# dropbox/lepton

Hardware: AMD Instinct MI355X
Metric: encode+decode MB/s (JPEG bytes/sec), bit-exact round trip (higher is better)
Workload: dtype int16/u8 (integer coder, no floating point)

## Files before the change

lepton_amd/csrc/lep_dec4.h:

```cpp
#pragma once
#include "lep_v3.h"
#include "lep_enc3.h"

namespace lep4 {
using namespace lep3;

#if LEP_ON_GPU && defined(LEP_MARKS)
#define LEP_MARK(name) __asm__ volatile("; MARK " name)
#elif LEP_ON_GPU && defined(LEP_PROF)
#define LEP_MARK(name) prof_stamp(lep4::prof_slot(name))
#else
#define LEP_MARK(name) ((void)0)
#endif
#if LEP_ON_GPU && (defined(LEP_DEC4_PAD_VALU) || defined(LEP_DEC4_PAD_SALU) || defined(LEP_DEC4_PAD_LDS))
#define LEP_PAD8(x) x x x x x x x x
WDEV void pad_block(uint32_t seed, const void* lds) {
    (void)seed; (void)lds;
#ifdef LEP_DEC4_PAD_VALU
    { uint32_t o; for (int i = 0; i < LEP_DEC4_PAD_VALU / 8; ++i) __asm__ volatile(LEP_PAD8("v_add_u32 %0, %1, %1\n") : "=v"(o) : "v"(seed)); }
#endif
#ifdef LEP_DEC4_PAD_SALU
    { uint32_t o; const uint32_t u = uni(seed); for (int i = 0; i < LEP_DEC4_PAD_SALU / 8; ++i) __asm__ volatile(LEP_PAD8("s_add_u32 %0, %1, %1\n") : "=s"(o) : "s"(u) : "scc"); }
#endif
#ifdef LEP_DEC4_PAD_LDS
// ... 238 lines not shown
#if !LEP_DEC4_REFILL_GROUPS
        if (count < 0) refill(b);
#else
        (void)b;
#endif
#ifdef LEP_DEC4_RANGE_LOW
        const uint32_t split = 1 + (((range - 1) * (pk & 255u)) >> 8);
        const uint32_t big = split << 24;
        uint32_t was = vhi;
        const uint32_t bit = was >= big ? 1u : 0u;
        vhi = bit ? was - big : was;
        range = bit ? range - split : split;
        const int shift = __builtin_clz(range) - 24;
#else
        const uint32_t big = ((uint32_t)(((uint64_t)(range - 0x01000000u) * (uint64_t)(pk << 24)) >> 32) & 0xff000000u) + 0x01000000u;
        uint32_t was = vhi;
        const uint32_t bit = was >= big ? 1u : 0u;
        vhi = bit ? was - big : was;
        range = bit ? range - big : big;
        const int shift = __builtin_clz(range);
#endif
#ifdef LEP_TRACE_GET
        LEP_TRACE_GET(pk & 255u, (int)bit);
#endif
        range <<= shift;
        const uint64_t v = pair64(vhi, vlo) << shift;
        vhi = (uint32_t)(v >> 32); vlo = (uint32_t)v;
        count -= shift;
#if LEP_ON_GPU && !defined(LEP_DEC4_PAIR_OR)
        __asm__ volatile("" : "+s"(was));
        return was >= big ? 1u : 0u;
#else
        return bit;
#endif
    }
};

#ifndef LEP_DEC4_PRIO
#define LEP_DEC4_PRIO 1
#endif
#if LEP_ON_GPU && LEP_DEC4_PRIO
#define LEP_PRIO_SERIAL(on_scalar_unit) __builtin_amdgcn_s_setprio((on_scalar_unit) ? 0 : 1)
#define LEP_PRIO_PARALLEL() __builtin_amdgcn_s_setprio(2)
#else
#define LEP_PRIO_SERIAL(on_scalar_unit) ((void)0)
#define LEP_PRIO_PARALLEL() ((void)0)
#endif
#ifndef LEP_DEC4_SCALAR
#define LEP_DEC4_SCALAR 2
#endif

#ifndef LEP_DEC4_WORD_PER_LANE
#define LEP_DEC4_WORD_PER_LANE 1
#endif

enum : int32_t { kRowsFresh = 0, kRowsRunning = 1, kRowsFinished = 2, kRowsFailed = 3 };
struct Dec4Resume {
    int32_t state, code;
    uint32_t idx, top;
    uint32_t vhi, vlo;
    int32_t count;
    uint32_t range, wi;
    uint32_t nbins;
    int32_t rows_done[3];
    int32_t fail_component, fail_y, fail_x;
};

struct RowsWalk {
    const Dec4Resume* rec; const uint32_t* lds_save;
    bool fresh;
    uint32_t idx, stop, total;
    int band;
    bool top[3];
    int rows_done[3];
    int state, fail_component, fail_y, fail_x;
};

template <int SCMASK>
struct Dec4WaveT {
    const ImageDev* img;
    uint32_t* model;
    Dec4Shared* sh;
    int comp, ci;
    BoolDec4 bc;
    uint32_t nbins;
#if LEP_ON_GPU && !defined(LEP_COUNT_BINS)
#define LEP_BINS(expr) ((void)0)
#else
#define LEP_BINS(expr) (expr)
#endif
#if LEP_ON_GPU && defined(LEP_PROF)
    uint64_t prof_last;
    unsigned long long* prof_out;
    int prof_cur;
    uint32_t prof_acc[20];
    template <int I> __device__ __forceinline__ void prof_add(uint32_t dt) { if (prof_cur == I) prof_acc[I] += dt; }
    __device__ __forceinline__ void prof_stamp(int slot) {
        const uint64_t t = __builtin_readcyclecounter();
        const uint32_t dt = (uint32_t)(t - prof_last);
        prof_last = t;
        prof_add<0>(dt); prof_add<1>(dt); prof_add<2>(dt); prof_add<3>(dt); prof_add<4>(dt); prof_add<5>(dt); prof_add<6>(dt);
        prof_add<7>(dt); prof_add<8>(dt); prof_add<9>(dt); prof_add<10>(dt); prof_add<11>(dt); prof_add<12>(dt); prof_add<13>(dt);
        prof_add<14>(dt); prof_add<15>(dt); prof_add<16>(dt); prof_add<17>(dt); prof_add<18>(dt);
        prof_cur = slot;
    }
    __device__ __forceinline__ void prof_begin(unsigned long long* out) {
// ... 178 lines not shown
#define LEP_SLOT(k, fld)                                                                                              \
        if (!((kAlways >> k) & 1)) { LANES(l) L(any) = (L(used) >> k) & 1; }                                           \
        if (((kAlways >> k) & 1) || lepwave::wave_ballot(any)) {                                                       \
            LANES(l) {                                                                                                \
                const uint32_t w = L(W).fld;                                                                          \
                const uint32_t u1 = ((uint32_t)(L(used) & L(bits)) >> k) & 1u, u0 = ((uint32_t)(L(used) & ~L(bits)) >> k) & 1u;   \
                const uint32_t w2 = w + (u0 | (u1 << 8));                                                             \
                const uint32_t f = w2 & 255u, t = (w2 >> 8) & 255u;                                                   \
                const uint32_t p = mul24_low(f, inv[f + t]);    \
                const uint32_t m = mul24(u0 | u1, 0xff0000u);                                                         \
                L(oldw) = w; L(low) = (f < t ? f : t) + ((u0 | u1) ^ 1u);    \
                L(W).fld = (p & m) | (w2 & ~m);                                                                       \
            }                                                                                                         \
            LANES(l) L(any) = L(low) == 0;                                                                            \
            if (lepwave::wave_ballot(any)) {                                                                          \
                LANES(l) if (L(low) == 0) L(W).fld = bupd_t(L(oldw), (uint32_t)(L(bits) >> k) & 1u, inv);             \
            }                                                                                                         \
        }
        LEP_SLOT(0, x) LEP_SLOT(1, y) LEP_SLOT(2, z) LEP_SLOT(3, w)
#undef LEP_SLOT
    }

    WDEV void adapt_words(uint32_t* W, const int* use, const int* obs) {
        const uint32_t* inv = sh->inv24;
        LV(int, wrapped); LV(uint32_t, oldw);
        LANES(l) {
            const uint32_t w = L(W);
            const uint32_t u = (uint32_t)L(use), u1 = u & (uint32_t)L(obs), u0 = u & ~(uint32_t)L(obs);
            const uint32_t w2 = w + (u0 | (u1 << 8));
            const uint32_t f = w2 & 255u, t = (w2 >> 8) & 255u;
            const uint32_t p = mul24_low(f, inv[f + t]);
            const uint32_t m = mul24(u, 0xff0000u);
            L(oldw) = w; L(wrapped) = (f < t ? f : t) + (u ^ 1u) == 0;
            L(W) = (p & m) | (w2 & ~m);
        }
        if (lepwave::wave_ballot(wrapped)) {
            LANES(l) if (L(wrapped)) L(W) = bupd_t(L(oldw), (uint32_t)L(obs), inv);
        }
    }
    static WDEV void regroup(const U4* G, const int* src, const int* slot, uint32_t* out) {
        LV(uint32_t, c0); LV(uint32_t, c1); LV(uint32_t, c2); LV(uint32_t, c3);
        LV(uint32_t, g0); LV(uint32_t, g1); LV(uint32_t, g2); LV(uint32_t, g3);
        LANES(l) { L(c0) = L(G).x; L(c1) = L(G).y; L(c2) = L(G).z; L(c3) = L(G).w; }
        lepwave::wave_gather(c0, src, g0); lepwave::wave_gather(c1, src, g1);
        lepwave::wave_gather(c2, src, g2); lepwave::wave_gather(c3, src, g3);
        LANES(l) { const int k = L(slot); L(out) = k == 0 ? L(g0) : (k == 1 ? L(g1) : (k == 2 ? L(g2) : L(g3))); }
    }
    WDEV void adapt_regrouped(const U4* G, const uint32_t* adr, const int* src, const int* slot, const int* use, const int* obs) {
        LV(uint32_t, Wd); LV(uint32_t, ad);
        regroup(G, src, slot, Wd);
        lepwave::wave_gather(adr, src, ad);
        adapt_words(Wd, use, obs);
        LANES(l) if (L(use)) model[L(ad) + (uint32_t)L(slot)] = L(Wd);
    }

    WDEV int round_nz(int nzbin_ctx) {
        LEP_MARK("nz_prefetch");
        LV(U4, W0); LV(uint32_t, a0); LV(uint32_t, PK0);
        LANES(l) {
            uint32_t adr = 0, pk = 0;
            if (l < 17) {
                int i, k;
                if (l < 3) { i = 5 - l; k = 0; } else if (l < 5) { i = 2; k = l - 3; } else if (l < 9) { i = 1; k = l - 5; } else { i = 0; k = l - 9; }
                adr = ctx_nz7(ci, nzbin_ctx) + (uint32_t)i * 32 + (uint32_t)k * 4;
                L(W0) = ld4(model + adr); pk = pack_probs(L(W0));
            }
            L(a0) = adr; L(PK0) = pk;
        }
        LEP_MARK("nz_serial"); LEP_PRIO_SERIAL((SCMASK & 1) != 0);
        int nz;
        {
            Serial<(SCMASK & 1) != 0> sr(*this);
            nz = sr.template tree<6>(PK0, 0);
            sr.done();
            LEP_BINS(nbins += 6);
        }
        LEP_MARK("nz_update"); LEP_PRIO_PARALLEL();
#if LEP_DEC4_WORD_PER_LANE
        {
            LV(int, src); LV(int, slot); LV(int, use); LV(int, ob);
            LANES(l) {
                const int t = l < 6 ? l : 0, i = 5 - t, prefix = nz >> (i + 1);
                L(src) = ((0x953210 >> (4 * t)) & 15) + (prefix >> 2); L(slot) = prefix & 3; L(use) = l < 6; L(ob) = (nz >> i) & 1;
            }
            adapt_regrouped(W0, a0, src, slot, use, ob);
        }
#else
        LV(int, u0); LV(int, b0);
        LANES(l) {
            int u = 0, b = 0;
            if (l < 17) {
                int i, k;
                if (l < 3) { i = 5 - l; k = 0; } else if (l < 5) { i = 2; k = l - 3; } else if (l < 9) { i = 1; k = l - 5; } else { i = 0; k = l - 9; }
                mask_tree(i, k, nz, u, b);
            }
            L(u0) = u; L(b0) = b;
        }
        adapt_group<3>(W0, u0, b0);
        LANES(l) if (L(u0)) st4(model + L(a0), L(W0));
#endif
        return nz;
    }

    WDEV void round_77(int& zz_io, int& left_io) {
        Dec4Shared& S = *sh;
        LEP_MARK("77_prefetch");
// ... 26 lines not shown
        {
            typedef Serial<(SCMASK & 2) != 0> SR;
            SR sr(*this);
            uint32_t sgw = SR::U(S.sign[ci * 48]);
            int pi = 0;
#pragma nounroll
            for (;;) {
                int lane = pi + 16 * cand;
                const int lane_end = pi_end + 16 * cand;
                uint32_t pkv;
                bool found = false;
#pragma nounroll
                for (;;) {
                    pkv = SR::U(lepwave::wave_read(PK0, lane));
                    LEP_BINS(++nbins);
                    if (SR::is(sr.get(pkv & 255) != 0)) { found = true; break; }
                    if (++lane >= lane_end) break;
                }
                pi = lane - 16 * cand;
                if (!found) break;
                zz = zz0 + pi;
                int len = sr.template unary_from<1, false>(pkv);
                if (len == 4) {
                    len = 4 + sr.template unary_from<0>(SR::U(pack_probs(vload4(model + ctx4_exp7(ci, nb0 - cand, zz, (int)uni(S.bsr[zz])) + kGS))));
                    if (len == 8) len = sr.unary_tail(ctx4_exp7(ci, nb0 - cand, zz, (int)uni(S.bsr[zz])));
                }
                LEP_BINS(nbins += (uint32_t)(2 * len - (len == 11)));
                const uint32_t pos = sr.get(sgw >> 16);
                sgw = sr.bupd(sgw, pos);
                --left;
                uint32_t v = 1u << (len - 1);
                if (len > 1) {
                    int b = len - 2;
                    if (b >= 4) {
                        const uint32_t rbase = ctx4_res(ci, (int)uni(S.a2r[zz]), nb0 - cand);
#pragma nounroll
                        for (; b >= 4; --b) v |= sr.global_bin(row_word(rbase, b)) << b;
                    }
                    v = sr.residual(SR::U(lepwave::wave_read(PK1, lane)), b, v);
                }
                S.here[zz] = (int16_t)(pos ? (int)v : -(int)v);
                ++pi;
                if (left == 0) break;
                cand = nb0 - nzbin_of(left);
                if (cand >= LEP_DEC4_CANDS || pi >= pi_end) break;
            }
            zz = zz0 + pi;
            sr.done();
            S.sign[ci * 48] = sgw;
        }
        LSYNC();
        LEP_MARK("77_update"); LEP_PRIO_PARALLEL();
        LV(int, nzw);
        LANES(l) L(nzw) = l < 16 && zz0 + l < zz && S.here[zz0 + l] != 0;
        const uint32_t nzmask = (uint32_t)lepwave::wave_ballot(nzw);
        LV(int, u0); LV(int, b0); LV(int, u1); LV(int, b1); LV(int, u2); LV(int, b2);
#if LEP_DEC4_WORD_PER_LANE
        LV(int, src); LV(int, slot);
        LANES(l) {
            int s = l, ua = 0, oa = 0, ub = 0, ob = 0, uc = 0, bcc = 0;
            const int pi = l & 15, k = l >> 4, p = zz0 + pi;
            if (p < zz) {
                const int left_at = left0 - __builtin_popcount(nzmask & ((1u << pi) - 1));
                const int c = left_at > 0 ? nb0 - (int)S.nzbin[left_at] : LEP_DEC4_CANDS;
                if (c < LEP_DEC4_CANDS) {
                    const int cf = S.here[p];
                    const int v = cf < 0 ? -cf : cf, len = bitlen((uint32_t)v);
                    s = pi + 16 * c;
                    ua = k <= len; oa = len != k;
                    ub = k <= len - 2; ob = (v >> k) & 1;
                    if (c == k) mask_exp(4, len, uc, bcc);
                }
            }
            L(src) = s; L(slot) = k; L(u0) = ua; L(b0) = oa; L(u1) = ub; L(b1) = ob; L(u2) = uc; L(b2) = bcc;
        }
        adapt_regrouped(W0, a0, src, slot, u0, b0);
        if (lepwave::wave_ballot(u1)) adapt_regrouped(W1, a1, src, slot, u1, b1);
#else
        LANES(l) {
            int ua = 0, ba = 0, ub = 0, bb = 0, uc = 0, bcc = 0;
            const int pi = l & 15, cand_l = l >> 4, p = zz0 + pi;
            if (L(ok) && p < zz) {
                const int left_at = left0 - __builtin_popcount(nzmask & ((1u << pi) - 1));
                if (left_at > 0 && nb0 - (int)S.nzbin[left_at] == cand_l) {
                    const int cf = S.here[p];
                    const int v = cf < 0 ? -cf : cf, len = bitlen((uint32_t)v);
                    mask_exp(0, len, ua, ba);
                    mask_res(len - 2, v, ub, bb);
                    mask_exp(4, len, uc, bcc);
                }
            }
            L(u0) = ua; L(b0) = ba; L(u1) = ub; L(b1) = bb; L(u2) = uc; L(b2) = bcc;
        }
        adapt_group<3>(W0, u0, b0);
        adapt_group<0>(W1, u1, b1);
        LANES(l) {
            if (L(u0)) st4(model + L(a0), L(W0));
            if (L(u1)) st4(model + L(a1), L(W1));
        }
#endif
        if (lepwave::wave_ballot(u2)) {
            LV(U4, W2);
            LANES(l) if (L(u2)) L(W2) = ld4(model + L(a0) + kGS);
            adapt_group<0>(W2, u2, b2);
            LANES(l) if (L(u2)) st4(model + L(a0) + kGS, L(W2));
        }
        LSYNC();
        zz_io = zz; left_io = left;
    }

    WDEV int round_edges(int nz, int eob_x, int eob_y, bool has_left, bool has_above) {
        Dec4Shared& S = *sh;
        LEP_MARK("edge_prefetch");
        LV(U4, W0); LV(U4, W1); LV(U4, W2); LV(uint32_t, a0); LV(uint32_t, a2); LV(uint32_t, PK0); LV(uint32_t, PK1); LV(uint32_t, PK2);
        LV(uint32_t, INFO);
        LANES(l) {
            uint32_t adr0 = 0, adr2 = 0, pk0 = 0, pk1 = 0, pk2 = 0, info = 0;
            if (l < 56) {
                const int e = l >= 28 ? 1 : 0, c = l - e * 28, j = S.cj[c], n = S.cn[c];
                const bool horizontal = e == 0;
                const int coord = horizontal ? j + 1 : (j + 1) * 8;
                const int32_t prior = S.eprior[e * 7 + j];
                const uint32_t ap = prior < 0 ? 0u - (uint32_t)prior : (uint32_t)prior;
                const int bsr = bitlen(ap > 1023 ? 1023 : ap);
                adr0 = ctx4_expx(ci, n, horizontal ? j : j + 7, bsr);
                adr2 = ctx4_res(ci, coord, n);
                L(W0) = ld4(model + adr0); L(W2) = ld4(model + adr2);
                pk0 = pack_probs(L(W0)); pk2 = pack_probs(L(W2));
                L(W1) = U4{0, 0, 0, 0};
                const int16_t p16 = (int16_t)prior;
                const int thr = S.thr[coord];
                const uint32_t tctx = (uint32_t)imin((int)((ap & 0xffff) >> thr), 255);
                info = (uint32_t)((ci * 4 + (p16 == 0 ? 0 : (p16 > 0 ? 1 : 2))) * 12 + bsr) | ((uint32_t)thr << 8) | (tctx << 16) |
                       ((uint32_t)bsr << 24) | ((S.eprior[14] >> (e * 7 + j)) & 1 ? 0x80000000u : 0u);
            } else if (l < 62) {
                const int e = l >= 59 ? 1 : 0, lv = l - 56 - 3 * e;
                adr0 = ctx_nzedge(e == 0, ci, e == 0 ? eob_x : eob_y, (nz + 3) / 7) + (uint32_t)(2 - lv) * 4;
                L(W0) = ld4(model + adr0); pk0 = pack_probs(L(W0));
            }
            L(a0) = adr0; L(a2) = adr2; L(PK0) = pk0; L(PK1) = pk1; L(PK2) = pk2; L(INFO) = info;
        }
        LSYNC();
        LEP_MARK("edge_serial"); LEP_PRIO_SERIAL((SCMASK & 4) != 0);
        int ne[2] = {0, 0}, rc = 0;
        typedef Serial<(SCMASK & 4) != 0> SR;
        SR sr(*this);
#pragma nounroll
        for (int e = 0; e < 2 && !rc; ++e) {
            const bool horizontal = e == 0;
            ne[e] = sr.template tree<3>(PK0, 56 + 3 * e);
            LEP_BINS(nbins += 3);
            int left = ne[e];
            if (!left) continue;
            const int a_off = horizontal ? 50 : 57;
            int lane = e * 28 + left - 1, step = 7;
#pragma nounroll
            for (;;) {
                if (SR::is(left > step)) {
#pragma nounroll
// ... 41 lines not shown
                    const int coord = horizontal ? j + 1 : (j + 1) * 8;
                    int len = sr.template unary_from<1, false>(pkv);
                    if (len == 4) {
                        len = 4 + sr.template unary_from<0>(SR::U(pack_probs(vload4(model + ctx4_expx(ci, left, horizontal ? j : j + 7, (int)((info >> 24) & 15)) + kGS))));
                        if (len == 8) len = sr.unary_tail(ctx4_expx(ci, left, horizontal ? j : j + 7, (int)((info >> 24) & 15)));
                    }
                    LEP_BINS(nbins += (uint32_t)(2 * len - (len == 11)));
                    const int sslot = (int)(info & 255);
                    const uint32_t sgw = SR::U(S.sign[sslot]);
                    const uint32_t pos = sr.get(sgw >> 16);
                    S.sign[sslot] = sr.bupd(sgw, pos);
                    uint32_t v = 1u << (len - 1);
                    if (len > 1) {
                        int b = len - 2;
                        const int thr = (int)((info >> 8) & 15);
                        if (b >= thr) {
                            const uint32_t Tt = ctx_thresh(ci, (int)((info >> 16) & 255), imin(len - thr, 7));
                            int sx = 1;
#pragma nounroll
                            for (; b >= thr; --b) {
                                const uint32_t bit = sr.global_bin(Tt + (uint32_t)sx);
                                v |= bit << b;
                                sx = imin((sx << 1) | (int)uni(bit), 127);
                            }
                        }
                        if (b >= 4) {
                            const uint32_t rbase = ctx4_res(ci, coord, left);
#pragma nounroll
                            for (; b >= 4; --b) v |= sr.global_bin(row_word(rbase, b)) << b;
                        }
                        v = sr.residual(SR::U(lepwave::wave_read(PK2, lane)), b, v);
                    }
                    S.here[a_off + j] = (int16_t)(pos ? (int)v : -(int)v);
                    --lane;
                    if (--left == 0) break;
                }
                lane += step;
                if (--step == 0) break;
            }
        }
        sr.done();
        LSYNC();
        if (rc) return rc;
        LEP_MARK("edge_update"); LEP_PRIO_PARALLEL();
        LV(int, enz);
        LANES(l) L(enz) = l >= 50 && S.here[l] != 0;
        const uint64_t em = lepwave::wave_ballot(enz);
        const uint32_t mh = (uint32_t)(em >> 50) & 0x7f, mv = (uint32_t)(em >> 57) & 0x7f;
        const int neh = ne[0], nev = ne[1];
        LV(int, u1); LV(int, b1); LV(int, u2); LV(int, b2);
#if !LEP_DEC4_WORD_PER_LANE
        LV(int, u0); LV(int, b0);
#endif
        LANES(l) {
            int ua = 0, ba = 0, ub = 0, bb = 0, uc = 0, bcc = 0;
            if (l < 56) {
                const int e = l >= 28 ? 1 : 0, c = l - e * 28, j = S.cj[c], n = S.cn[c];
                const uint32_t mk = e ? mv : mh;
                const int left_at = (e ? nev : neh) - __builtin_popcount(mk & ((1u << j) - 1));
                if (left_at == n) {
                    const int cf = S.here[(e ? 57 : 50) + j];
                    const int v = cf < 0 ? -cf : cf, len = bitlen((uint32_t)v);
#if !LEP_DEC4_WORD_PER_LANE
                    mask_exp(0, len, ua, ba);
#endif
                    mask_exp(4, len, ub, bb);
                    mask_res(imin(len - 2, (int)S.thr[e ? (j + 1) * 8 : j + 1] - 1), v, uc, bcc);
                }
            }
#if !LEP_DEC4_WORD_PER_LANE
            else if (l < 62) {
                const int e = l >= 59 ? 1 : 0, lv = l - 56 - 3 * e;
                mask_tree(2 - lv, 0, e ? nev : neh, ua, ba);
            }
            L(u0) = ua; L(b0) = ba;
#else
            (void)ua; (void)ba;
#endif
            L(u1) = ub; L(b1) = bb; L(u2) = uc; L(b2) = bcc;
        }
#if LEP_DEC4_WORD_PER_LANE
        {
            LV(int, src); LV(int, slot); LV(int, use); LV(int, ob);
            LANES(l) {
                int s = l, k = l & 3, u = 0, o = 0;
                if (l < 56) {
                    const int q = l >> 2, e = q >= 7 ? 1 : 0, j = q - 7 * e;
                    const int left_at = (e ? nev : neh) - __builtin_popcount((e ? mv : mh) & ((1u << j) - 1));
                    if (left_at >= 1 && left_at <= 7 - j) {
                        const int cf = S.here[(e ? 57 : 50) + j];
                        const int v = cf < 0 ? -cf : cf, len = bitlen((uint32_t)v);
                        s = e * 28 + ((j * (15 - j)) >> 1) + left_at - 1;
                        u = k <= len; o = len != k;
                    }
                } else if (l < 62) {
                    const int e = l >= 59 ? 1 : 0, i = 2 - (l - 56 - 3 * e), value = e ? nev : neh;
                    k = (value >> (i + 1)) & 3; u = 1; o = (value >> i) & 1;
                }
                L(src) = s; L(slot) = k; L(use) = u; L(ob) = o;
            }
            adapt_regrouped(W0, a0, src, slot, use, ob);
        }
#else
        adapt_group<3>(W0, u0, b0);
        LANES(l) if (L(u0)) st4(model + L(a0), L(W0));
#endif
        if (lepwave::wave_ballot(u1)) {
            LANES(l) if (L(u1)) L(W1) = ld4(model + L(a0) + kGS);
            adapt_group<0>(W1, u1, b1);
            LANES(l) if (L(u1)) st4(model + L(a0) + kGS, L(W1));
        }
        if (lepwave::wave_ballot(u2)) {
            adapt_group<0>(W2, u2, b2);
            LANES(l) if (L(u2)) st4(model + L(a2), L(W2));
        }
        LSYNC();
        return 0;
    }

    WDEV void round_dc(int pred, int a, int b17, int sctx) {
        Dec4Shared& S = *sh;
        LEP_MARK("dc_prefetch");
        LV(U4, W0); LV(uint32_t, a0); LV(uint32_t, PK0); LV(uint32_t, RW);
        LANES(l) {
            uint32_t adr = 0, pk = 0, rw = 0;
            if (l < 3) { adr = ctx_expdc(a, b17) + (uint32_t)l * 4; L(W0) = ld4(model + adr); pk = pack_probs(L(W0)); }
            else if (l < 13) rw = S.resdc[a * 12 + (l - 3)];
            L(a0) = adr; L(PK0) = pk; L(RW) = rw;
        }
        LEP_MARK("dc_serial"); LEP_PRIO_SERIAL((SCMASK & 8) != 0);
        const int sslot = ci * 48 + sctx;
        typedef Serial<(SCMASK & 8) != 0> SR;
        SR sr(*this);
        int len = sr.template unary_from<0>(SR::U(lepwave::wave_read(PK0, 0)));
        if (len == 4) {
            len += sr.template unary_from<0>(SR::U(lepwave::wave_read(PK0, 1)));
            if (len == 8) {
                uint32_t pk = SR::U(lepwave::wave_read(PK0, 2));
                sr.ensure();
#pragma nounroll
                for (; len < 11; ++len) { if (!SR::is(sr.get_raw(pk & 255) != 0)) break; pk >>= 8; }
            }
        }
        LEP_BINS(nbins += (uint32_t)(len ? 2 * len + 1 - (len == 11) : 1));
        uint32_t v = 0, pos = 1;
        if (len) {
            const uint32_t sgw = SR::U(S.sign[sslot]);
            pos = sr.get(sgw >> 16);
            S.sign[sslot] = sr.bupd(sgw, pos);
            v = 1u << (len - 1);
#pragma nounroll
            for (int i = len - 2; i >= 0; --i) v |= sr.get(SR::U(lepwave::wave_read(RW, 3 + i)) >> 16) << i;
        }
        sr.done();
        v = vec(v);
        int d = (int16_t)(pos ? (int)v : -(int)v);
        int dc = d + pred;
        dc = dc < -1024 ? dc + 2049 : dc;
        dc = dc > 1024 ? dc - 2049 : dc;
        S.here[49] = (int16_t)dc;
        LSYNC();
        LEP_MARK("dc_update"); LEP_PRIO_PARALLEL();
        LV(uint32_t, VV);
        LANES(l) L(VV) = v;
#if LEP_DEC4_WORD_PER_LANE
        {
            LV(int, src); LV(int, slot); LV(int, use); LV(int, ob); LV(uint32_t, Wd); LV(uint32_t, ad); LV(uint32_t, rg);
            LANES(l) {
                int s = l, k = 0, u = 0, o = 0;
                if (l < 11) { s = l >> 2; k = l & 3; u = l <= len; o = len != l; }
                else if (l < 21) { s = l - 8; u = l - 11 <= len - 2; o = (int)((L(VV) >> (l - 11)) & 1u); }
                L(src) = s; L(slot) = k; L(use) = u; L(ob) = o;
            }
            regroup(W0, src, slot, Wd);
            lepwave::wave_gather(RW, src, rg);
            lepwave::wave_gather(a0, src, ad);
            LANES(l) if (l >= 11) L(Wd) = L(rg);
            adapt_words(Wd, use, ob);
            LANES(l) if (L(use)) {
                if (l < 11) model[L(ad) + (uint32_t)L(slot)] = L(Wd);
                else S.resdc[a * 12 + (l - 11)] = L(Wd);
            }
        }
#else
        LV(int, u0); LV(int, b0);
        LANES(l) {
            int u = 0, b = 0;
            if (l < 3) mask_exp(l * 4, len, u, b);
            L(u0) = u; L(b0) = b;
        }
        adapt_group<7>(W0, u0, b0);
        LANES(l) {
            if (L(u0)) st4(model + L(a0), L(W0));
            if (l >= 3 && l < 13 && l - 3 <= len - 2) S.resdc[a * 12 + (l - 3)] = bupd_t(L(RW), (L(VV) >> (l - 3)) & 1u, S.inv24);
        }
#endif
        LSYNC();
    }

    WDEV int decode_block(bool has_left, bool has_above) {
        Dec4Shared& S = *sh;
        LEP_MARK("prologue");
        LANES(l) {
            S.here[l] = 0;
            if (l < 49) {
                int prior;
                if (has_left && has_above) prior = (uint16_t)((iabs(S.left[l]) + iabs(S.above[l])) * 13 + 6 * iabs(S.aleft[l])) >> 5;
                else if (has_left) prior = (int16_t)iabs(S.left[l]);
                else if (has_above) prior = (int16_t)iabs(S.above[l]);
                else prior = 0;
                S.bsr[l] = (uint8_t)bitlen((uint32_t)imin(iabs(prior), 1023));
            }
        }
        int nzctx = 0;
        if (has_left && has_above) nzctx = (S.ns_above.nz + S.ns_left.nz + 2) / 4;
        else if (has_above) nzctx = (S.ns_above.nz + 1) / 2;
        else if (has_left) nzctx = (S.ns_left.nz + 1) / 2;
        const int nzbin_ctx = (int)uni((uint32_t)nzbin_of(nzctx));
        LSYNC();

        const int nz = round_nz(nzbin_ctx);
        if (nz > 49) return 7;
        {
            int zz = 0, left = nz;
#pragma nounroll
            while (zz < 49 && left > 0) round_77(zz, left);
        }
        LEP_MARK("lakhani");
        int eob_x, eob_y;
        {
            LV(int, tx); LV(int, ty); LV(int, badf);
            LANES(l) {
                int ex = 0, ey = 0, bad = 0;
                if (l < 49 && S.here[l] != 0) { const int coord = S.a2r[l]; ex = coord & 7; ey = coord >> 3; }
                if (l < 14) {
                    const bool hz = l < 7;
                    const int j = hz ? l : l - 7;
                    const int coord = hz ? j + 1 : (j + 1) * 8;
                    int32_t prior = 0;
                    if (hz ? has_above : has_left) {
                        const int16_t* nbr = hz ? S.above : S.left;
                        const int32_t* icos = hz ? S.icos_x + coord * 8 : S.icos_y + coord;
                        const int step = hz ? 8 : 1;
                        if (icos[0] != 0) {
                            uint32_t acc = (uint32_t)(int32_t)nbr[S.r2a[coord]] * (uint32_t)icos[0];
                            for (int i = 1; i < 8; ++i) {
                                int32_t xi = S.here[S.r2a[coord + i * step]], ai = nbr[S.r2a[coord + i * step]];
                                int32_t term = (i & 1) ? xi + ai : xi - ai;
                                acc -= (uint32_t)icos[i] * (uint32_t)term;
                            }
                            prior = div_by((int32_t)acc, (uint32_t)(hz ? S.icos_x[j] : S.icos_y[j]), DivBy::shift_of((uint32_t)icos[0]));
                        } else bad = 1;
                    }
                    S.eprior[l] = prior;
                }
                L(tx) = ex; L(ty) = ey; L(badf) = bad;
            }
            eob_x = lepwave::wave_max(tx); eob_y = lepwave::wave_max(ty);
            const uint64_t badmask = lepwave::wave_ballot(badf);
            LANES(l) if (l == 0) S.eprior[14] = (int32_t)(uint32_t)badmask;
            LSYNC();
        }
        {
            const int rc = round_edges(nz, eob_x, eob_y, has_left, has_above);
            if (rc) return rc;
        }
        LEP_MARK("idct_dcpred");
        idct_rows();
        int pred, a, b17, sctx;
        {
            LV(int, emin); LV(int, emax); LV(int, s0); LV(int, s1); LV(int, tmp);
            LANES(l) {
                int ev = 0, have = 0;
                if (l < 8 && has_left) { have = 1; ev = (int16_t)(S.ns_left.vert[l] - half16(LEP_PIX(S, l, 0) - LEP_PIX(S, l, 1)) - (LEP_PIX(S, l, 0) + 1024)); }
                if (l >= 8 && l < 16 && has_above) { const int i = l - 8; have = 1; ev = (int16_t)(S.ns_above.horiz[i] - half16(LEP_PIX(S, 0, i) - LEP_PIX(S, 1, i)) - (LEP_PIX(S, 0, i) + 1024)); }
                L(emax) = have ? ev : -0x7fffffff;
                L(emin) = have ? -ev : -0x7fffffff;
                L(s0) = l < 8 ? ev : 0;
                L(s1) = (l >= 8 && l < 16) ? ev : 0;
            }
            const int mx = lepwave::wave_max(emax), mn = -lepwave::wave_max(emin);
            const int sumL = lepwave::wave_sum(s0), sumA = lepwave::wave_sum(s1);
            int32_t avgmed = 0, unc = 0, unc2 = 0;
            if (has_left || has_above) {
                int sum0 = has_left ? sumL : sumA, sum1 = (has_left && has_above) ? sumA : sum0;
                avgmed = (sum0 + sum1) >> 1;
                unc = (mx - mn) >> 3;
                sum0 -= avgmed; sum1 -= avgmed;
                unc2 = (iabs(sum0) < iabs(sum1) ? sum0 : sum1) >> 3;
            }
            const uint32_t dc_shift = (uint32_t)S.icos_y[7];
            pred = ((dc_shift == 32 ? avgmed : div_by(avgmed, (uint32_t)S.icos_x[7], dc_shift)) + 4) >> 3;
            a = imin(bitlen((uint32_t)iabs(unc) & 0xffff), 11);
            b17 = imin(bitlen((uint32_t)iabs(unc2) & 0xffff), 16);
            sctx = unc2 >= 0 ? (unc2 == 0 ? 3 : 2) : 1;
        }
        round_dc(pred, a, b17, sctx);
        LEP_MARK("publish");
        pad_block((uint32_t)pred, sh);
        LANES(l) {
            if (l < 16) {
                const int i = l & 7;
                const int dcq = S.here[49] * (int)S.q[0];
                if (l < 8) S.ns_here.horiz[i] = (int16_t)(dcq + LEP_PIX(S, 7, i) + 1024 + half16(LEP_PIX(S, 7, i) - LEP_PIX(S, 6, i)));
                else S.ns_here.vert[i] = (int16_t)(dcq + LEP_PIX(S, i, 7) + 1024 + half16(LEP_PIX(S, i, 7) - LEP_PIX(S, i, 6)));
            }
            if (l == 16) S.ns_here.nz = nz;
        }
        LSYNC();
        return 0;
    }

    template <bool ROWS = false>
    WDEV int run(const ImageDev* image, const SegDev& seg, uint32_t* model_words, NSum* ns, Dec4Shared* shared, const uint8_t* stream,
                 uint32_t len, RowsWalk* rw = nullptr) {
        img = image; model = model_words; sh = shared; nbins = 0;
        LEP_PRIO_PARALLEL();
        init_tables();
        if (ROWS && !rw->fresh) resume_stream(stream, len, *rw);
        else bc.init_stream(stream, len);
        bool top[3] = {true, true, true};
        if (ROWS) for (int c = 0; c < 3; ++c) top[c] = rw->top[c];
        for (uint32_t idx = ROWS ? rw->idx : 0;; ++idx) {
            RowSpec r = row_spec(image, idx);
            if (r.done) break;
            if (r.luma_y >= seg.y1 && !seg.is_last) break;
            if (ROWS) if (idx >= rw->stop) { rw->state = kRowsRunning; rw->idx = idx; break; }
            if (r.skip) continue;
            if (r.luma_y < seg.y0) continue;
            if (ROWS) if (rw->stop == 0xffffffffu && rw->band > 0) rw->stop = (idx / rw->total + (uint32_t)rw->band) * rw->total;
            stage_component(r.component);
            const int w = img->width[comp], yb = r.curr_y;
            int16_t* row = img->blocks[comp] + (int64_t)yb * w * 64;
            const bool has_above = !top[comp];
            const int16_t* arow = has_above ? row - (int64_t)w * 64 : nullptr;
            NSum* nrow = ns + img->ns_offset[comp] + (yb & 1) * w;
            const NSum* narow = ns + img->ns_offset[comp] + ((yb & 1) ^ 1) * w;
            top[comp] = false;
            LV(int16_t, nxt_above); LV(uint32_t, nxt_ns);
            LANES(l) {
                L(nxt_above) = has_above ? arow[l] : (int16_t)0;
                L(nxt_ns) = (has_above && l < (int)(sizeof(NSum) / 4)) ? ((const uint32_t*)&narow[0])[l] : 0u;
            }
            const int coded_here = (int)img->coded_blocks[comp] - yb * w;
            const int x_end = imin(w, coded_here < 1 ? 1 : coded_here);
            for (int x = 0; x < x_end; ++x) {
                LEP_MARK("staging");
        LANES(l) {
                    if (x) { sh->left[l] = sh->here[l]; sh->aleft[l] = sh->above[l]; }
                    if (l < (int)(sizeof(NSum) / 4)) {
                        if (x) ((uint32_t*)&sh->ns_left)[l] = ((const uint32_t*)&sh->ns_here)[l];
                        if (has_above) ((uint32_t*)&sh->ns_above)[l] = L(nxt_ns);
                    }
                }
                LSYNC();
                LANES(l) {
                    if (has_above) sh->above[l] = L(nxt_above);
                    if (has_above && x + 1 < x_end) {
                        L(nxt_above) = arow[(int64_t)(x + 1) * 64 + l];
                        if (l < (int)(sizeof(NSum) / 4)) L(nxt_ns) = ((const uint32_t*)&narow[x + 1])[l];
                    }
                }
                LSYNC();
                int rc = decode_block(x > 0, has_above);
                if (ROWS) if (rc) { rw->state = kRowsFailed; rw->fail_component = comp; rw->fail_y = yb; rw->fail_x = x; }
                if (rc) return rc;
                LEP_MARK("store");
        LANES(l) {
                    row[(int64_t)x * 64 + l] = sh->here[l];
                    if (l < (int)(sizeof(NSum) / 4)) ((uint32_t*)&nrow[x])[l] = ((const uint32_t*)&sh->ns_here)[l];
                }
            }
            if (ROWS) for (int c = 0; c < 3; ++c) { if (c == comp) { rw->rows_done[c] = yb + 1; rw->top[c] = false; } }
        }
        return 0;
    }

    WDEV void resume_stream(const uint8_t* stream, uint32_t len, const RowsWalk& rw) {
        const uint32_t mis = (uint32_t)((uintptr_t)stream & 3);
        bc.words = reinterpret_cast<const uint32_t*>(stream - mis);
        bc.first = mis; bc.end = mis + len;
        bc.vhi = vec(rw.rec->vhi); bc.vlo = vec(rw.rec->vlo); bc.count = (int)vec((uint32_t)rw.rec->count); bc.range = vec(rw.rec->range);
        bc.wi = rw.rec->wi;
        bc.raw = bc.fetch(bc.wi);
        nbins = rw.rec->nbins;
        LANES(l) {
            for (int d = l; d < kSignWords; d += 64) sh->sign[d] = rw.lds_save[d];
            for (int d = l; d < kResDcWords; d += 64) sh->resdc[d] = rw.lds_save[kSignWords + d];
        }
        LSYNC();
    }

    WDEV void run_rows(const ImageDev* image, const SegDev& seg, uint32_t* model_words, NSum* ns, Dec4Shared* shared, const uint8_t* stream,
                       uint32_t len, Dec4Resume* rec, uint32_t* lds_save, int band_mcu_rows) {
        RowsWalk rw;
        rw.rec = rec; rw.lds_save = lds_save;
        rw.fresh = rec->state == kRowsFresh;
        rw.idx = 0; rw.stop = 0xffffffffu; rw.total = 0; rw.band = band_mcu_rows;
        for (int i = 0; i < 3 && i < image->ncomp; ++i) rw.total += (uint32_t)image->height[i] / (uint32_t)image->mcu_rows;
        for (int c = 0; c < 3; ++c) { rw.top[c] = true; rw.rows_done[c] = 0; }
        rw.state = kRowsFinished; rw.fail_component = -1; rw.fail_y = -1; rw.fail_x = -1;
        if (!rw.fresh) {
            rw.idx = rec->idx;
            for (int c = 0; c < 3; ++c) { rw.top[c] = ((rec->top >> c) & 1u) != 0; rw.rows_done[c] = rec->rows_done[c]; }
            if (band_mcu_rows > 0) rw.stop = (rw.idx / rw.total + (uint32_t)band_mcu_rows) * rw.total;
        }
        const int code = run<true>(image, seg, model_words, ns, shared, stream, len, &rw);
        LSYNC();
        if (rw.state == kRowsRunning) {
            LANES(l) {
                for (int d = l; d < kSignWords; d += 64) lds_save[d] = sh->sign[d];
                for (int d = l; d < kResDcWords; d += 64) lds_save[kSignWords + d] = sh->resdc[d];
            }
        }
#if LEP_ON_GPU
        if (threadIdx.x != 0) return;
#endif
// ... 12 lines not shown
```

lepton_amd/csrc/lep_v3.h:

```cpp
#pragma once
#include "lep_core.h"
#include "lep_wave.h"

namespace lep3 {
using namespace lepdev;

enum : uint32_t {
    kNz7x7 = 0,
    kNz1x8 = kNz7x7 + 2 * 26 * 6 * 32,
    kNz8x1 = kNz1x8 + 2 * 8 * 8 * 3 * 4,
    kExpDc = kNz8x1 + 2 * 8 * 8 * 3 * 4,
    kRes = kExpDc + 12 * 17 * 12,
    kExpX = kRes + 2 * 64 * 10 * 12,
    kExp7 = kExpX + 2 * 10 * 15 * 12 * 12,
    kThresh = kExp7 + 2 * 10 * 49 * 12 * 12,
    kModelWords = kThresh + 2 * 256 * 8 * 128
};
static_assert(kModelWords == 739472 && kModelWords % 4 == 0, "v3 model layout");
constexpr int kSignWords = 96, kResDcWords = 144;

struct U4 { uint32_t x, y, z, w; };

WDEV uint32_t prob_of(uint32_t f, uint32_t t) {
#if LEP_ON_GPU
    const uint32_t n = f << 8, d = f + t;
    uint32_t q = (uint32_t)((float)n * __builtin_amdgcn_rcpf((float)d));
    const int r = (int)n - (int)(q * d);
    q += r >= (int)d ? 1u : 0u;
    q -= r < 0 ? 1u : 0u;
    return q;
#else
    return (f << 8) / (f + t);
#endif
}

WDEV uint32_t uni(uint32_t v) {
#if LEP_ON_GPU
    return (uint32_t)__builtin_amdgcn_readfirstlane((int)v);
#else
    return v;
#endif
}
WDEV uint32_t vec(uint32_t v) {
#if LEP_ON_GPU
    __asm__ volatile("" : "+v"(v));
#endif
    return v;
}
WDEV uint32_t uload(const uint32_t* p) {
#if LEP_ON_GPU
    uintptr_t a = (uintptr_t)p;
    __asm__ volatile("" : "+v"(a));
    return uni(*reinterpret_cast<const uint32_t*>(a));
#else
    return *p;
#endif
}

struct InvTable {
    uint32_t v[512];
    constexpr InvTable() : v() {
        for (int d = 2; d < 512; ++d) v[d] = (uint32_t)((0x100000000ull + (uint64_t)d - 1) / (uint64_t)d);
    }
};
#ifdef __HIP_DEVICE_COMPILE__
__constant__ static const InvTable kInv = InvTable();
#else
static const InvTable kInv = InvTable();
#endif
WDEV uint32_t bupd_s(uint32_t w, int obs) {
    uint32_t f = (w & 255) + (uint32_t)(obs ^ 1), t = ((w >> 8) & 255) + (uint32_t)obs;
    if (__builtin_expect((f | t) > 255, 0)) {
        const uint32_t f0 = w & 255, t0 = (w >> 8) & 255;
        if ((obs ? f0 : t0) == 1) return (w & 0xffff) | ((obs ? 0u : 255u) << 16);
        f = obs ? (1 + f0) >> 1 : 129u;
        t = obs ? 129u : (1 + t0) >> 1;
    }
    const uint32_t p = (uint32_t)(((uint64_t)(f << 8) * kInv.v[f + t]) >> 32);
    return f | (t << 8) | (p << 16);
}

WDEV uint32_t bupd(uint32_t w, int obs) {
    uint32_t f = w & 255, t = (w >> 8) & 255;
    const uint32_t mine = obs ? t : f, other = obs ? f : t;
    if (mine == 255) {
        if (other == 1) return (w & 0xffff) | ((obs ? 0u : 255u) << 16);
        f = (1 + f) >> 1; t = (1 + t) >> 1;
        if (obs) t = 129; else f = 129;
    } else {
        if (obs) ++t; else ++f;
    }
    return f | (t << 8) | (prob_of(f, t) << 16);
}

WDEV U4 ld4(const uint32_t* p) { U4 v; __builtin_memcpy(&v, __builtin_assume_aligned(p, 16), 16); return v; }
// ... 113 lines not shown
```

Measured before the change: 1637.

## Use wave-uniform branch flags, branchless lane selects, and word-per-lane adapts

Wraps per-block flags (has_left, has_above, loop bounds, return codes) in wave-uniform casts so the compiler can emit scalar branches instead of divergent exec-mask branches. Per-lane setup loops are rewritten as branchless selects with clamped indices. The second and third adaptation groups in the nz and edge rounds switch to a one-word-per-lane reload-and-adapt path in place of 4-wide group loads. The extra unconditional LDS reads and the changed adapt scheduling may add work on some lanes, and bit-exactness depends on the rewritten masks matching the old ones.

```diff
diff --git a/lepton_amd/csrc/lep_dec4.h b/lepton_amd/csrc/lep_dec4.h
--- a/lepton_amd/csrc/lep_dec4.h
+++ b/lepton_amd/csrc/lep_dec4.h
@@ -314,6 +314,23 @@
 
 #ifndef LEP_DEC4_WORD_PER_LANE
 #define LEP_DEC4_WORD_PER_LANE 1
+#endif
+#ifndef LEP_DEC4_UNIFORM_TESTS
+#define LEP_DEC4_UNIFORM_TESTS 1
+#endif
+#ifndef LEP_DEC4_LANE_SELECTS
+#define LEP_DEC4_LANE_SELECTS 1
+#endif
+#ifndef LEP_DEC4_WORD_PER_LANE_2
+#define LEP_DEC4_WORD_PER_LANE_2 1
+#endif
+#define LEP_DEC4_WPL2 (LEP_DEC4_WORD_PER_LANE_2 && LEP_DEC4_WORD_PER_LANE && LEP_DEC4_LANE_SELECTS)
+#if LEP_DEC4_UNIFORM_TESTS
+#define LEP_UFLAG(c) uflag(c)
+#define LEP_UINT(v) unii(v)
+#else
+#define LEP_UFLAG(c) (c)
+#define LEP_UINT(v) (v)
 #endif
 
 enum : int32_t { kRowsFresh = 0, kRowsRunning = 1, kRowsFinished = 2, kRowsFailed = 3 };
@@ -598,6 +615,17 @@
         lepwave::wave_gather(adr, src, ad);
         adapt_words(Wd, use, obs);
         LANES(l) if (L(use)) model[L(ad) + (uint32_t)L(slot)] = L(Wd);
+    }
+    WDEV void adapt_reloaded(const uint32_t* adr, const int* src, const int* slot, const int* use, const int* obs, uint32_t off) {
+        LV(uint32_t, Wd); LV(uint32_t, ad);
+        lepwave::wave_gather(adr, src, ad);
+        LANES(l) {
+            L(ad) += off + (uint32_t)L(slot);
+            L(Wd) = 0;
+            if (L(use)) L(Wd) = model[L(ad)];
+        }
+        adapt_words(Wd, use, obs);
+        LANES(l) if (L(use)) model[L(ad)] = L(Wd);
     }
 
     WDEV int round_nz(int nzbin_ctx) {
@@ -730,11 +758,38 @@
         LSYNC();
         LEP_MARK("77_update"); LEP_PRIO_PARALLEL();
         LV(int, nzw);
+#if LEP_DEC4_LANE_SELECTS
+        {
+            const int seen = imin(16, zz - zz0);
+            LANES(l) L(nzw) = (l < seen) & (S.here[(zz0 + l) & 63] != 0);
+        }
+#else
         LANES(l) L(nzw) = l < 16 && zz0 + l < zz && S.here[zz0 + l] != 0;
+#endif
         const uint32_t nzmask = (uint32_t)lepwave::wave_ballot(nzw);
         LV(int, u0); LV(int, b0); LV(int, u1); LV(int, b1); LV(int, u2); LV(int, b2);
 #if LEP_DEC4_WORD_PER_LANE
         LV(int, src); LV(int, slot);
+#if LEP_DEC4_LANE_SELECTS
+        LANES(l) {
+            const int pi = l & 15, k = l >> 4, p = zz0 + pi;
+            const int left_at = left0 - __builtin_popcount(nzmask & ((1u << pi) - 1));
+            const int c = nb0 - (int)S.nzbin[left_at > 0 ? left_at : 0];
+            const int cf = S.here[p];
+            const int v = cf < 0 ? -cf : cf, len = bitlen((uint32_t)v);
+            const int on = (p < zz) & (left_at > 0) & (c < LEP_DEC4_CANDS);
+            L(src) = on ? pi + 16 * c : l; L(slot) = k;
+            L(u0) = on & (k <= len); L(b0) = len != k;
+            L(u1) = on & (k <= len - 2); L(b1) = (v >> k) & 1;
+#if LEP_DEC4_WPL2
+            L(u2) = on & (4 + k <= imin(len, 10)); L(b2) = len != 4 + k;
+#else
+            int uc, bcc;
+            mask_exp(4, len, uc, bcc);
+            L(u2) = (on & (c == k)) ? uc : 0; L(b2) = bcc;
+#endif
+        }
+#else
         LANES(l) {
             int s = l, ua = 0, oa = 0, ub = 0, ob = 0, uc = 0, bcc = 0;
             const int pi = l & 15, k = l >> 4, p = zz0 + pi;
@@ -752,6 +807,7 @@
             }
             L(src) = s; L(slot) = k; L(u0) = ua; L(b0) = oa; L(u1) = ub; L(b1) = ob; L(u2) = uc; L(b2) = bcc;
         }
+#endif
         adapt_regrouped(W0, a0, src, slot, u0, b0);
         if (lepwave::wave_ballot(u1)) adapt_regrouped(W1, a1, src, slot, u1, b1);
 #else
@@ -777,12 +833,16 @@
             if (L(u1)) st4(model + L(a1), L(W1));
         }
 #endif
+#if LEP_DEC4_WPL2
+        if (lepwave::wave_ballot(u2)) adapt_reloaded(a0, src, slot, u2, b2, kGS);
+#else
         if (lepwave::wave_ballot(u2)) {
             LV(U4, W2);
             LANES(l) if (L(u2)) L(W2) = ld4(model + L(a0) + kGS);
             adapt_group<0>(W2, u2, b2);
             LANES(l) if (L(u2)) st4(model + L(a0) + kGS, L(W2));
         }
+#endif
         LSYNC();
         zz_io = zz; left_io = left;
     }
@@ -930,6 +990,22 @@
 #if !LEP_DEC4_WORD_PER_LANE
         LV(int, u0); LV(int, b0);
 #endif
+#if LEP_DEC4_WPL2
+#elif LEP_DEC4_LANE_SELECTS && LEP_DEC4_WORD_PER_LANE
+        LANES(l) {
+            const int lc = l < 56 ? l : 0;
+            const int e = lc >= 28 ? 1 : 0, c = lc - e * 28, j = S.cj[c], n = S.cn[c];
+            const uint32_t mk = e ? mv : mh;
+            const int left_at = (e ? nev : neh) - __builtin_popcount(mk & ((1u << j) - 1));
+            const int cf = S.here[(e ? 57 : 50) + j];
+            const int v = cf < 0 ? -cf : cf, len = bitlen((uint32_t)v);
+            int ub, bb, uc, bcc;
+            mask_exp(4, len, ub, bb);
+            mask_res(imin(len - 2, (int)S.thr[e ? (j + 1) * 8 : j + 1] - 1), v, uc, bcc);
+            const int on = (l < 56) & (left_at == n);
+            L(u1) = on ? ub : 0; L(b1) = bb; L(u2) = on ? uc : 0; L(b2) = bcc;
+        }
+#else
         LANES(l) {
             int ua = 0, ba = 0, ub = 0, bb = 0, uc = 0, bcc = 0;
             if (l < 56) {
@@ -957,9 +1033,30 @@
 #endif
             L(u1) = ub; L(b1) = bb; L(u2) = uc; L(b2) = bcc;
         }
+#endif
 #if LEP_DEC4_WORD_PER_LANE
         {
             LV(int, src); LV(int, slot); LV(int, use); LV(int, ob);
+#if LEP_DEC4_LANE_SELECTS
+            LANES(l) {
+                const int q = imin(l >> 2, 13), e = q >= 7 ? 1 : 0, j = q - 7 * e;
+                const int left_at = (e ? nev : neh) - __builtin_popcount((e ? mv : mh) & ((1u << j) - 1));
+                const int cf = S.here[(e ? 57 : 50) + j];
+                const int v = cf < 0 ? -cf : cf, len = bitlen((uint32_t)v);
+                const int kp = l & 3;
+                const int vis = (l < 56) & ((uint32_t)(left_at - 1) < (uint32_t)(7 - j));
+                const int tr = (l >= 56) & (l < 62), t = tr ? l - 56 : 0;
+                const int te = t >= 3 ? 1 : 0, i = 2 - (t - 3 * te), value = te ? nev : neh;
+                L(src) = vis ? e * 28 + ((j * (15 - j)) >> 1) + left_at - 1 : l;
+                L(slot) = tr ? (value >> (i + 1)) & 3 : kp;
+                L(use) = tr | (vis & (kp <= len));
+                L(ob) = tr ? (value >> i) & 1 : len != kp;
+#if LEP_DEC4_WPL2
+                L(u1) = vis & (4 + kp <= imin(len, 10)); L(b1) = len != 4 + kp;
+                L(u2) = vis & (kp <= imin(len - 2, (int)S.thr[e ? (j + 1) * 8 : j + 1] - 1)); L(b2) = (v >> kp) & 1;
+#endif
+            }
+#else
             LANES(l) {
                 int s = l, k = l & 3, u = 0, o = 0;
                 if (l < 56) {
@@ -977,12 +1074,18 @@
                 }
                 L(src) = s; L(slot) = k; L(use) = u; L(ob) = o;
             }
+#endif
             adapt_regrouped(W0, a0, src, slot, use, ob);
+#if LEP_DEC4_WPL2
+            if (lepwave::wave_ballot(u1)) adapt_reloaded(a0, src, slot, u1, b1, kGS);
+            if (lepwave::wave_ballot(u2)) adapt_regrouped(W2, a2, src, slot, u2, b2);
+#endif
         }
 #else
         adapt_group<3>(W0, u0, b0);
         LANES(l) if (L(u0)) st4(model + L(a0), L(W0));
 #endif
+#if !LEP_DEC4_WPL2
         if (lepwave::wave_ballot(u1)) {
             LANES(l) if (L(u1)) L(W1) = ld4(model + L(a0) + kGS);
             adapt_group<0>(W1, u1, b1);
@@ -992,6 +1095,7 @@
             adapt_group<0>(W2, u2, b2);
             LANES(l) if (L(u2)) st4(model + L(a2), L(W2));
         }
+#endif
         LSYNC();
         return 0;
     }
@@ -1003,7 +1107,14 @@
         LANES(l) {
             uint32_t adr = 0, pk = 0, rw = 0;
             if (l < 3) { adr = ctx_expdc(a, b17) + (uint32_t)l * 4; L(W0) = ld4(model + adr); pk = pack_probs(L(W0)); }
+#if LEP_DEC4_LANE_SELECTS
+            {
+                const uint32_t r = S.resdc[a * 12 + imin(l < 3 ? 0 : l - 3, 9)];
+                rw = ((l >= 3) & (l < 13)) ? r : 0u;
+            }
+#else
             else if (l < 13) rw = S.resdc[a * 12 + (l - 3)];
+#endif
             L(a0) = adr; L(PK0) = pk; L(RW) = rw;
         }
         LEP_MARK("dc_serial"); LEP_PRIO_SERIAL((SCMASK & 8) != 0);
@@ -1076,9 +1187,30 @@
         LSYNC();
     }
 
-    WDEV int decode_block(bool has_left, bool has_above) {
+    static WDEV uint8_t bsr_of(int prior) { return (uint8_t)bitlen((uint32_t)imin(iabs(prior), 1023)); }
+    WDEV int decode_block(bool has_left_, bool has_above_) {
         Dec4Shared& S = *sh;
+        const bool has_left = LEP_UFLAG(has_left_), has_above = LEP_UFLAG(has_above_);
         LEP_MARK("prologue");
+#if LEP_DEC4_UNIFORM_TESTS
+        int nzctx;
+        {
+            const int nz_above = unii(S.ns_above.nz), nz_left = unii(S.ns_left.nz);
+            if (has_left && has_above) {
+                LANES(l) { S.here[l] = 0; if (LEP_DEC4_LANE_SELECTS || l < 49) S.bsr[l] = bsr_of((uint16_t)((iabs(S.left[l]) + iabs(S.above[l])) * 13 + 6 * iabs(S.aleft[l])) >> 5); }
+                nzctx = (int)((uint32_t)(nz_above + nz_left + 2) >> 2);
+            } else if (has_left) {
+                LANES(l) { S.here[l] = 0; if (LEP_DEC4_LANE_SELECTS || l < 49) S.bsr[l] = bsr_of((int16_t)iabs(S.left[l])); }
+                nzctx = (int)((uint32_t)(nz_left + 1) >> 1);
+            } else if (has_above) {
+                LANES(l) { S.here[l] = 0; if (LEP_DEC4_LANE_SELECTS || l < 49) S.bsr[l] = bsr_of((int16_t)iabs(S.above[l])); }
+                nzctx = (int)((uint32_t)(nz_above + 1) >> 1);
+            } else {
+                LANES(l) { S.here[l] = 0; if (LEP_DEC4_LANE_SELECTS || l < 49) S.bsr[l] = 0; }
+                nzctx = 0;
+            }
+        }
+#else
         LANES(l) {
             S.here[l] = 0;
             if (l < 49) {
@@ -1094,6 +1226,7 @@
         if (has_left && has_above) nzctx = (S.ns_above.nz + S.ns_left.nz + 2) / 4;
         else if (has_above) nzctx = (S.ns_above.nz + 1) / 2;
         else if (has_left) nzctx = (S.ns_left.nz + 1) / 2;
+#endif
         const int nzbin_ctx = (int)uni((uint32_t)nzbin_of(nzctx));
         LSYNC();
 
@@ -1110,7 +1243,15 @@
             LV(int, tx); LV(int, ty); LV(int, badf);
             LANES(l) {
                 int ex = 0, ey = 0, bad = 0;
+#if LEP_DEC4_LANE_SELECTS
+                {
+                    const int coord = S.a2r[l];
+                    const int in = (l < 49) & (S.here[l] != 0);
+                    ex = in ? coord & 7 : 0; ey = in ? coord >> 3 : 0;
+                }
+#else
                 if (l < 49 && S.here[l] != 0) { const int coord = S.a2r[l]; ex = coord & 7; ey = coord >> 3; }
+#endif
                 if (l < 14) {
                     const bool hz = l < 7;
                     const int j = hz ? l : l - 7;
@@ -1150,8 +1291,20 @@
             LV(int, emin); LV(int, emax); LV(int, s0); LV(int, s1); LV(int, tmp);
             LANES(l) {
                 int ev = 0, have = 0;
+#if LEP_DEC4_LANE_SELECTS
+                {
+                    const int i = l & 7;
+                    const bool lf = (l & 8) == 0;
+                    const int p0 = S.pix[lf ? i : i * 8], p1 = S.pix[lf ? 8 + i : i * 8 + 1];
+                    const int16_t* nsp = lf ? S.ns_left.vert : S.ns_above.horiz;
+                    const int nsv = nsp[i];
+                    have = (l < 16) & (lf ? (int)has_left : (int)has_above);
+                    ev = have ? (int)(int16_t)(nsv - half16(p0 - p1) - (p0 + 1024)) : 0;
+                }
+#else
                 if (l < 8 && has_left) { have = 1; ev = (int16_t)(S.ns_left.vert[l] - half16(LEP_PIX(S, l, 0) - LEP_PIX(S, l, 1)) - (LEP_PIX(S, l, 0) + 1024)); }
                 if (l >= 8 && l < 16 && has_above) { const int i = l - 8; have = 1; ev = (int16_t)(S.ns_above.horiz[i] - half16(LEP_PIX(S, 0, i) - LEP_PIX(S, 1, i)) - (LEP_PIX(S, 0, i) + 1024)); }
+#endif
                 L(emax) = have ? ev : -0x7fffffff;
                 L(emin) = have ? -ev : -0x7fffffff;
                 L(s0) = l < 8 ? ev : 0;
@@ -1176,6 +1329,18 @@
         round_dc(pred, a, b17, sctx);
         LEP_MARK("publish");
         pad_block((uint32_t)pred, sh);
+#if LEP_DEC4_LANE_SELECTS
+        static_assert(__builtin_offsetof(NSum, vert) == 0 && __builtin_offsetof(NSum, horiz) == 16 && __builtin_offsetof(NSum, nz) == 32, "publish writes NSum as half words");
+        LANES(l) {
+            const int i = l & 7;
+            const bool hz = (l & 8) == 0;
+            const int pa = S.pix[hz ? i * 8 + 7 : 56 + i], pb = S.pix[hz ? i * 8 + 6 : 48 + i];
+            const int dcq = S.here[49] * (int)S.q[0];
+            const int edge = dcq + pa + 1024 + half16(pa - pb);
+            const int val = l < 16 ? edge : (l == 16 ? nz : nz >> 16);
+            if (l < 18) ((int16_t*)&S.ns_here)[l < 16 ? l ^ 8 : l] = (int16_t)val;
+        }
+#else
         LANES(l) {
             if (l < 16) {
                 const int i = l & 7;
@@ -1185,6 +1350,7 @@
             }
             if (l == 16) S.ns_here.nz = nz;
         }
+#endif
         LSYNC();
         return 0;
     }
@@ -1210,7 +1376,7 @@
             stage_component(r.component);
             const int w = img->width[comp], yb = r.curr_y;
             int16_t* row = img->blocks[comp] + (int64_t)yb * w * 64;
-            const bool has_above = !top[comp];
+            const bool has_above = LEP_UFLAG(!top[comp]);
             const int16_t* arow = has_above ? row - (int64_t)w * 64 : nullptr;
             NSum* nrow = ns + img->ns_offset[comp] + (yb & 1) * w;
             const NSum* narow = ns + img->ns_offset[comp] + ((yb & 1) ^ 1) * w;
@@ -1221,9 +1387,29 @@
                 L(nxt_ns) = (has_above && l < (int)(sizeof(NSum) / 4)) ? ((const uint32_t*)&narow[0])[l] : 0u;
             }
             const int coded_here = (int)img->coded_blocks[comp] - yb * w;
-            const int x_end = imin(w, coded_here < 1 ? 1 : coded_here);
+            const int x_end = LEP_UINT(imin(w, coded_here < 1 ? 1 : coded_here));
             for (int x = 0; x < x_end; ++x) {
                 LEP_MARK("staging");
+#if LEP_DEC4_UNIFORM_TESTS
+                const bool first = uflag(x == 0), more = uflag(has_above && x + 1 < x_end);
+                if (!first) { LANES(l) { sh->left[l] = sh->here[l]; sh->aleft[l] = sh->above[l]; } }
+                {
+                    const uint32_t* ns_from = first ? (const uint32_t*)&sh->ns_left : (const uint32_t*)&sh->ns_here;
+                    LANES(l) {
+                        sh->above[l] = L(nxt_above);
+                        if (l < (int)(sizeof(NSum) / 4)) { ((uint32_t*)&sh->ns_left)[l] = ns_from[l]; ((uint32_t*)&sh->ns_above)[l] = L(nxt_ns); }
+                    }
+                }
+                LSYNC();
+                if (more) {
+                    LANES(l) {
+                        L(nxt_above) = arow[(int64_t)(x + 1) * 64 + l];
+                        if (l < (int)(sizeof(NSum) / 4)) L(nxt_ns) = ((const uint32_t*)&narow[x + 1])[l];
+                    }
+                }
+                LSYNC();
+                int rc = unii(decode_block(!first, has_above));
+#else
         LANES(l) {
                     if (x) { sh->left[l] = sh->here[l]; sh->aleft[l] = sh->above[l]; }
                     if (l < (int)(sizeof(NSum) / 4)) {
@@ -1241,6 +1427,7 @@
                 }
                 LSYNC();
                 int rc = decode_block(x > 0, has_above);
+#endif
                 if (ROWS) if (rc) { rw->state = kRowsFailed; rw->fail_component = comp; rw->fail_y = yb; rw->fail_x = x; }
                 if (rc) return rc;
                 LEP_MARK("store");
diff --git a/lepton_amd/csrc/lep_v3.h b/lepton_amd/csrc/lep_v3.h
--- a/lepton_amd/csrc/lep_v3.h
+++ b/lepton_amd/csrc/lep_v3.h
@@ -41,6 +41,8 @@
     return v;
 #endif
 }
+WDEV bool uflag(bool c) { return uni(c ? 1u : 0u) != 0; }
+WDEV int unii(int v) { return (int)uni((uint32_t)v); }
 WDEV uint32_t vec(uint32_t v) {
 #if LEP_ON_GPU
     __asm__ volatile("" : "+v"(v));
```

Result: faster. 1673 (median of 6 runs) (+2.2%).
